# YonkaMayonkaZ/NCF

Measured on NVIDIA B200. Metric: NeuMF train samples/s, higher is better.
Workload: dtype f32

## Files before the change

ncf_b200/csrc/tile_umma.cu:

```cuda
#include <algorithm>
#include <cstdlib>

#include "common.cuh"
#include "tile_params.cuh"

namespace {

constexpr int kTile = 128;
constexpr uint32_t kHiMask = 0xffffe000u;
constexpr int kProducerWarps = 8;
constexpr int kLoaderWarp = 17;
constexpr int kGemmThreads = 576;
constexpr int kMaxStages = 4;

enum { EPI_RELU_STORE = 0, EPI_PREDICT = 1, EPI_PREDICT_TRAIN = 2, EPI_MASK_STORE = 3, EPI_SCATTER = 4 };

struct GemmArgs {
  int K;
  int N;
  int n_total;
  int passes;
  int layer;
  int gather;
  int stages;
  const float* a;
  const float* b_img;
  const float* bias;
  float* out;
  const float* mask_src;
};

struct WgradJob {
  int k, mb, nb, cta0, nctas;
  int S;
};
struct WgradArgs {
  int njobs, passes;
  WgradJob job[12];
};

__device__ __forceinline__ uint32_t smem_u32(const void* p) { return (uint32_t)__cvta_generic_to_shared(p); }

__device__ __forceinline__ void mbar_init(uint64_t* b, uint32_t count) {
  asm volatile("mbarrier.init.shared::cta.b64 [%0], %1;" ::"r"(smem_u32(b)), "r"(count));
}
__device__ __forceinline__ void mbar_arrive(uint64_t* b) {
  asm volatile("mbarrier.arrive.shared::cta.b64 _, [%0];" ::"r"(smem_u32(b)) : "memory");
}
__device__ __forceinline__ void mbar_expect_tx(uint64_t* b, uint32_t bytes) {
  asm volatile("mbarrier.arrive.expect_tx.shared::cta.b64 _, [%0], %1;" ::"r"(smem_u32(b)), "r"(bytes) : "memory");
}
__device__ __forceinline__ void mbar_wait(uint64_t* b, uint32_t parity) {
  const uint32_t addr = smem_u32(b);
  for (uint32_t spin = 0; spin < (1u << 26); ++spin) {
    uint32_t done;
#ifdef NCF_MBAR_POLL
    asm volatile(
        "{\n\t.reg .pred p;\n\tmbarrier.test_wait.parity.shared::cta.b64 p, [%1], %2;\n\tselp.u32 %0, 1, 0, p;\n\t}"
        : "=r"(done) : "r"(addr), "r"(parity) : "memory");
#else
    asm volatile(
        "{\n\t.reg .pred p;\n\tmbarrier.try_wait.parity.shared::cta.b64 p, [%1], %2;\n\tselp.u32 %0, 1, 0, p;\n\t}"
        : "=r"(done) : "r"(addr), "r"(parity) : "memory");
#endif
    if (done) return;
  }
  __trap();
}
__device__ __forceinline__ bool mbar_test_warp(uint64_t* b, uint32_t parity) {
  uint32_t done = 0;
  if ((threadIdx.x & 31) == 0)
    asm volatile(
        "{\n\t.reg .pred p;\n\tmbarrier.test_wait.parity.shared::cta.b64 p, [%1], %2;\n\tselp.u32 %0, 1, 0, p;\n\t}"
        : "=r"(done) : "r"(smem_u32(b)), "r"(parity) : "memory");
  return __shfl_sync(0xffffffffu, done, 0) != 0;
}
__device__ __forceinline__ void mbar_wait_warp(uint64_t* b, uint32_t parity) {
  if ((threadIdx.x & 31) == 0) mbar_wait(b, parity);
  __syncwarp();
}
__device__ __forceinline__ void mbar_arrive_warp(uint64_t* b) {
  __syncwarp();
  if ((threadIdx.x & 31) == 0) mbar_arrive(b);
}
__device__ __forceinline__ void bulk_g2s(void* dst, const void* src, uint32_t bytes, uint64_t* bar) {
  asm volatile("cp.async.bulk.shared::cluster.global.mbarrier::complete_tx::bytes [%0], [%1], %2, [%3];"
               ::"r"(smem_u32(dst)), "l"(src), "r"(bytes), "r"(smem_u32(bar)) : "memory");
}
__device__ __forceinline__ void cp_async16_zfill(void* dst, const void* src, bool valid) {
  asm volatile("cp.async.cg.shared.global [%0], [%1], 16, %2;" ::"r"(smem_u32(dst)), "l"(src), "r"(valid ? 16 : 0) : "memory");
}
__device__ __forceinline__ void fence_async_smem() { asm volatile("fence.proxy.async.shared::cta;" ::: "memory"); }
__device__ __forceinline__ void tc_fence_before() { asm volatile("tcgen05.fence::before_thread_sync;" ::: "memory"); }
__device__ __forceinline__ void tc_fence_after() { asm volatile("tcgen05.fence::after_thread_sync;" ::: "memory"); }
__device__ __forceinline__ void tc_commit(uint64_t* bar) {
  asm volatile("tcgen05.commit.cta_group::1.mbarrier::arrive::one.shared::cluster.b64 [%0];" ::"r"(smem_u32(bar)) : "memory");
}
__device__ __forceinline__ void tc_mma(uint32_t d_tmem, uint64_t da, uint64_t db, uint32_t idesc, uint32_t accumulate) {
  asm volatile(
      "{\n\t.reg .pred p;\n\tsetp.ne.b32 p, %4, 0;\n\t"
      "tcgen05.mma.cta_group::1.kind::tf32 [%0], %1, %2, %3, p;\n\t}"
      ::"r"(d_tmem), "l"(da), "l"(db), "r"(idesc), "r"(accumulate) : "memory");
}
__device__ __forceinline__ void tc_ld32(uint32_t taddr, float (&v)[32]) {
  uint32_t r[32];
  asm volatile(
      "tcgen05.ld.sync.aligned.32x32b.x32.b32 "
      "{%0,%1,%2,%3,%4,%5,%6,%7,%8,%9,%10,%11,%12,%13,%14,%15,"
      "%16,%17,%18,%19,%20,%21,%22,%23,%24,%25,%26,%27,%28,%29,%30,%31}, [%32];"
      : "=r"(r[0]), "=r"(r[1]), "=r"(r[2]), "=r"(r[3]), "=r"(r[4]), "=r"(r[5]), "=r"(r[6]), "=r"(r[7]),
        "=r"(r[8]), "=r"(r[9]), "=r"(r[10]), "=r"(r[11]), "=r"(r[12]), "=r"(r[13]), "=r"(r[14]), "=r"(r[15]),
        "=r"(r[16]), "=r"(r[17]), "=r"(r[18]), "=r"(r[19]), "=r"(r[20]), "=r"(r[21]), "=r"(r[22]), "=r"(r[23]),
        "=r"(r[24]), "=r"(r[25]), "=r"(r[26]), "=r"(r[27]), "=r"(r[28]), "=r"(r[29]), "=r"(r[30]), "=r"(r[31])
      : "r"(taddr));
  asm volatile("tcgen05.wait::ld.sync.aligned;" ::: "memory");
#pragma unroll
  for (int j = 0; j < 32; ++j) v[j] = __uint_as_float(r[j]);
}

__device__ __forceinline__ uint64_t make_desc(uint32_t addr, uint32_t lbo, uint32_t sbo, uint32_t layout) {
  uint64_t d = (uint64_t)(layout & 7) << 61;
  d |= (uint64_t)((addr >> 4) & 0x3fff);
  d |= (uint64_t)((lbo >> 4) & 0x3fff) << 16;
  d |= (uint64_t)((sbo >> 4) & 0x3fff) << 32;
  d |= (uint64_t)1 << 46;
  return d;
}
__device__ __forceinline__ uint32_t make_idesc(int m, int n, int a_mn, int b_mn) {
  uint32_t d = 0;
  d |= 1u << 4;
  d |= 2u << 7;
  d |= 2u << 10;
  d |= (uint32_t)a_mn << 15;
  d |= (uint32_t)b_mn << 16;
  d |= (uint32_t)(n >> 3) << 17;
  d |= (uint32_t)(m >> 4) << 24;
  return d;
}

__device__ __forceinline__ void split4(const float4 x, float4& hi, float4& lo) {
  hi.x = __uint_as_float(__float_as_uint(x.x) & kHiMask);
  hi.y = __uint_as_float(__float_as_uint(x.y) & kHiMask);
  hi.z = __uint_as_float(__float_as_uint(x.z) & kHiMask);
  hi.w = __uint_as_float(__float_as_uint(x.w) & kHiMask);
  lo = make_float4(x.x - hi.x, x.y - hi.y, x.z - hi.z, x.w - hi.w);
}

__device__ __forceinline__ float warp_colsum32(float (&v)[32], int lane) {
#pragma unroll
  for (int o = 16; o > 0; o >>= 1) {
    const bool upper = (lane & o) != 0;
#pragma unroll
    for (int i = 0; i < o; ++i) {
      const float send = upper ? v[i] : v[i + o];
      const float keep = upper ? v[i + o] : v[i];
      v[i] = keep + __shfl_xor_sync(0xffffffffu, send, o);
    }
  }
  return v[0];
}

__device__ __forceinline__ void named_bar(int id, int count) {
  asm volatile("bar.sync %0, %1;" ::"r"(id), "r"(count) : "memory");
}

__global__ void umma_weight_images_kernel(const TileParams p) {
  const int k = blockIdx.y >> 1, dir = blockIdx.y & 1;
  const int kin = p.W[k], nout = p.W[k + 1];
  const int rows = dir ? kin : nout, K = dir ? nout : kin;
  const int panels = (K + 31) / 32;
  const float* w = p.w[k];
  float* img = dir ? p.wsplit_b[k] : p.wsplit_f[k];
  const int64_t total = (int64_t)panels * rows * 32;
  for (int64_t idx = blockIdx.x * (int64_t)blockDim.x + threadIdx.x; idx < total;
       idx += (int64_t)gridDim.x * blockDim.x) {
    const int cc = (int)(idx & 31);
    const int r = (int)((idx >> 5) % rows);
    const int pi = (int)((idx >> 5) / rows);
    const int c = pi * 32 + cc;
    float x = 0.f;
    if (c < K) x = dir ? w[(int64_t)c * kin + r] : w[(int64_t)r * kin + c];
    const float hi = __uint_as_float(__float_as_uint(x) & kHiMask);
    const int64_t off = (int64_t)pi * 2 * rows * 32 + (int64_t)r * 32 + ((((cc >> 2) ^ (r & 7)) << 2) | (cc & 3));
    img[off] = hi;
    img[off + (int64_t)rows * 32] = x - hi;
  }
}
// ... 711 lines not shown
          } else if (TRAIN && ok && p.dlogit_in == nullptr) {
            pre_label = p.label[row];
            if (p.teacher != nullptr) pre_teacher = p.teacher[row];
          }
        }
        mbar_wait_warp(&bars.acc_ready[gi & 1], n_acc[gi & 1] & 1);
        ++n_acc[gi & 1];
        tc_fence_after();
        if (G.kind == 0 && G.k + 1 == L && hf == 1) bars.xch[q * 32 + lane] = gd;
        const bool zero_late = (gi + 1 == g.ng) && G.d_col == g.gemm[0].d_col;
        if (gi + 1 == g.ng) {
          if (!zero_late) {
            zero_cols(g.gemm[0].d_col, g.gemm[0].N);
            tc_wait_st();
          }
        } else if (g.gemm[gi + 1].new_operand) {
          for (int gj = gi + 1; gj < g.ng && (gj == gi + 1 || !g.gemm[gj].new_operand); ++gj)
            zero_cols(g.gemm[gj].d_col, g.gemm[gj].N);
          tc_wait_st();
          tc_fence_before();
          mbar_arrive_warp(&bars.opnd_ready);
        }
        const int N = G.N, k = G.k;
        const int nchunk = N >> 5;
        const int c_begin = (nchunk >= 2) ? hf * (nchunk / 2) * 32 : 0;
        const int c_end = (nchunk >= 2) ? (hf + 1) * (nchunk / 2) * 32 : (hf == 0 ? N : 0);
        if (G.kind == 0 && k + 1 == L) {
          const int trow = q * 32 + lane;
          if (hf == 0) {
            const float* bias = p.b[k];
            float acc = 0.f;
            for (int c0 = 0; c0 < N; c0 += 32) {
              tc_ld32(lane_addr + g.hcol[L] + c0, v);
#pragma unroll
              for (int j = 0; j < 32; ++j)
                acc = fmaf(__ldg(&p.pw[mlp_off + c0 + j]), fmaxf(v[j] + __ldg(&bias[c0 + j]), 0.f), acc);
            }
            named_bar(1 + q, 64);
            float x = acc + bars.xch[trow] + __ldg(p.pb);
            if (bad) x = __int_as_float(0x7fc00000);
            if (valid && p.logits != nullptr) p.logits[row] = x;
            if (TRAIN) {
              float ls = 0.f;
              if (ok && p.dlogit_in != nullptr) {
                dl = p.dlogit_in[row];
              } else if (ok) {
                const SampleLoss r = sample_loss(x, pre_label, p.teacher != nullptr, pre_teacher, p.alpha, p.invB);
                ls = r.loss;
                dl = r.dlogit;
              }
              bars.xch[trow] = dl;
              mbar_arrive_warp(&bars.dl_ready);
              const float ls_w = warp_sum(ls), dl_w = warp_sum(dl);
              if (lane == 0) {
                if (p.loss_accum != nullptr) atomicAdd(p.loss_accum, (double)ls_w * (double)p.invB);
                atomicAdd(&bars.pg[p.predict_size], dl_w);
              }
              for (int c0 = 0; c0 < N; c0 += 32) {
                tc_ld32(lane_addr + g.hcol[L] + c0, v);
                float z[32];
#pragma unroll
                for (int j = 0; j < 32; ++j) {
                  const float h = fmaxf(v[j] + __ldg(&bias[c0 + j]), 0.f);
                  z[j] = (h > 0.f) ? dl * __ldg(&p.pw[mlp_off + c0 + j]) : 0.f;
                  v[j] = dl * h;
                }
                tc_st32(lane_addr + g.hcol[L] + c0, z);
                const float s = warp_colsum32(v, lane);
                atomicAdd(&bars.pg[mlp_off + c0 + lane], s);
                if (g.passes == 3) {
#pragma unroll
                  for (int j = 0; j < 32; ++j) v[j] = lo_of(z[j]);
                  tc_st32(lane_addr + g.lcol[L] + c0, v);
                }
                quad8_transpose(z, lane);
                tc_wait_st();
                tc_fence_before();
                mbar_arrive_warp(&bars.panel_ready[c0 >> 5]);
                store_rows_t(z, p.delta[L], N, row - lane, p.B, c0, lane);
              }
            }
          } else {
            named_bar(1 + q, 64);
          }
        } else if (G.kind == 0) {
          const int kk = k + 1;
          const float* bias = p.b[k];
          for (int c0 = c_begin; c0 < c_end; c0 += 32) {
            tc_ld32(lane_addr + g.hcol[kk] + c0, v);
#pragma unroll
            for (int j = 0; j < 32; ++j) v[j] = fmaxf(v[j] + __ldg(&bias[c0 + j]), 0.f);
            tc_st32(lane_addr + g.hcol[kk] + c0, v);
            if (g.passes == 3) {
              float lo[32];
#pragma unroll
              for (int j = 0; j < 32; ++j) lo[j] = lo_of(v[j]);
              tc_st32(lane_addr + g.lcol[kk] + c0, lo);
            }
            if (TRAIN) quad8_transpose(v, lane);
            tc_wait_st();
            tc_fence_before();
            mbar_arrive_warp(&bars.panel_ready[c0 >> 5]);
            if (TRAIN) store_rows_t(v, p.act[kk], N, row - lane, p.B, c0, lane);
          }

        } else if (TRAIN && k > 0) {
          for (int c0 = c_begin; c0 < c_end; c0 += 32) {
            float x[32];
            tc_ld32(lane_addr + g.lcol[k] + c0, v);
            tc_ld32(lane_addr + g.hcol[k] + c0, x);
#pragma unroll
            for (int j = 0; j < 32; ++j) v[j] = (x[j] > 0.f) ? v[j] : 0.f;
            tc_st32(lane_addr + g.lcol[k] + c0, v);
            if (g.passes == 3) {
#pragma unroll
              for (int j = 0; j < 32; ++j) x[j] = lo_of(v[j]);
              tc_st32(lane_addr + g.hcol[k] + c0, x);
            }
            quad8_transpose(v, lane);
            tc_wait_st();
            tc_fence_before();
            mbar_arrive_warp(&bars.panel_ready[c0 >> 5]);
            store_rows_t(v, p.delta[k], N, row - lane, p.B, c0, lane);
          }
        } else if (TRAIN) {
          for (int c0 = c_begin; c0 < c_end; c0 += 32) {
            tc_ld32(lane_addr + G.d_col + c0, v);
            quad8_transpose(v, lane);
            const int col = G.row0 + c0;
            const bool to_user = col < dmlp;
            const int64_t my_idx = ok ? (to_user ? u : it) : -1;
            float* tab = (to_user ? p.gum + col : p.gim + (col - dmlp)) + 4 * (lane & 7);
#pragma unroll
            for (int i = 0; i < 8; ++i) {
              const int64_t idx = __shfl_sync(0xffffffffu, my_idx, (lane & ~7) + i);
              if (idx >= 0) red_add4(tab + idx * dmlp, make_float4(v[4 * i], v[4 * i + 1], v[4 * i + 2], v[4 * i + 3]));
            }
          }
        }
        if (zero_late) zero_cols(g.gemm[0].d_col, g.gemm[0].N);
        tc_wait_st();
        tc_fence_before();
        if (gi + 1 == g.ng) mbar_arrive_warp(&bars.tile_done);
      }
    }
  }
  tc_fence_before();
  __syncthreads();
  if (TRAIN)
    for (int i = tid; i <= p.predict_size; i += kTowerThreads) atomicAdd(&p.gt[p.pw_off + i], bars.pg[i]);
  if (warp == 8) asm volatile("tcgen05.dealloc.cta_group::1.sync.aligned.b32 %0, 512;" ::"r"(tmem));
}

constexpr int kWgProducerWarps = 8;
constexpr int kWgProducers = kWgProducerWarps * 32;
constexpr int kWgradThreads = kWgProducers + 96;

constexpr int kWgStages = 2;
struct WgradBars {
  uint64_t full[kWgStages], empty[kWgStages], acc_full;
  uint32_t tmem_base;
  float db[128];
};

__device__ __forceinline__ uint32_t mn_offset(int s, int fo, int S) {
  const int panel = fo >> 5, cc = fo & 31;
  return (uint32_t)(panel * (S * 128) + s * 128 + (((cc >> 3) ^ (s & 3)) << 5) + ((cc & 7) << 2));
}

__global__ void __launch_bounds__(kWgradThreads, 1)
umma_wgrad_kernel(const __grid_constant__ TileParams p, const __grid_constant__ WgradArgs g) {
  extern __shared__ __align__(1024) uint8_t smem_raw[];
  __shared__ WgradBars bars;
  uint8_t* smem = reinterpret_cast<uint8_t*>((reinterpret_cast<uintptr_t>(smem_raw) + 1023) & ~(uintptr_t)1023);
  const int tid = threadIdx.x, warp = tid >> 5, lane = tid & 31;
  int ji = 0;
  while (ji + 1 < g.njobs && (int)blockIdx.x >= g.job[ji + 1].cta0) ++ji;
  const WgradJob job = g.job[ji];
  const int k = job.k, kin = p.W[k], nout = p.W[k + 1];
  const int MB = min(128, nout - job.mb * 128), NB = min(256, kin - job.nb * 256);
  const int local = (int)blockIdx.x - job.cta0;
  const int S = job.S;
  const int64_t nchunks = (p.B + S - 1) / S;
  const uint32_t a_img = (uint32_t)MB * S * 4, b_img = (uint32_t)NB * S * 4;
  const uint32_t stage_bytes = 2 * a_img + 2 * b_img;
  const int64_t my_chunks = (local < nchunks) ? (nchunks - local + job.nctas - 1) / job.nctas : 0;

  if (tid == 0) {
    const int nm = (g.passes == 3) ? 3 : 1;
    for (int s = 0; s < kWgStages; ++s) { mbar_init(&bars.full[s], kWgProducerWarps); mbar_init(&bars.empty[s], nm); }
    mbar_init(&bars.acc_full, nm);
    asm volatile("fence.mbarrier_init.release.cluster;" ::: "memory");
  }
  if (tid < 128) bars.db[tid] = 0.f;
  if (warp == kWgProducerWarps) {
    asm volatile("tcgen05.alloc.cta_group::1.sync.aligned.shared::cta.b32 [%0], 256;" ::"r"(smem_u32(&bars.tmem_base)));
    asm volatile("tcgen05.relinquish_alloc_permit.cta_group::1.sync.aligned;");
  }
  tc_fence_before();
  __syncthreads();
  tc_fence_after();
  const uint32_t tmem = bars.tmem_base;
  if (warp < kWgProducerWarps) {
    float z[32];
#pragma unroll
    for (int j = 0; j < 32; ++j) z[j] = 0.f;
    for (int c0 = (warp >> 2) * 128; c0 < (warp >> 2) * 128 + 128; c0 += 32)
      tc_st32(tmem + ((uint32_t)((warp & 3) * 32) << 16) + c0, z);
    tc_wait_st();
  }
  tc_fence_before();
  __syncthreads();
  tc_fence_after();

  if (warp < kWgProducerWarps) {
    const int t = tid, d = p.d;
    const float* delta = p.delta[k + 1];
    const float* actk = (k > 0) ? p.act[k] : nullptr;
    const int pa = MB >> 2, pb = NB >> 2;
    const int na = S * pa / kWgProducers, nbp = S * pb / kWgProducers;
    const int ca = t % pa, sa0 = t / pa, sas = kWgProducers / pa;
    const int cb = t % pb, sb0 = t / pb, sbs = kWgProducers / pb;
    float4 dbsum = make_float4(0.f, 0.f, 0.f, 0.f);
    const int fo = job.nb * 256 + cb * 4;
    const bool from_user = fo < d;
    const int64_t* idx_src = from_user ? p.user : p.item;
    const float* tab = from_user ? p.eum + fo : p.eim + (fo - d);
    const int64_t idx_lim = from_user ? p.U : p.I;
    int64_t idx_even[8], idx_odd[8];
    auto issue_idx = [&](int64_t ci, int64_t (&idxv)[8]) {
      const int64_t row0 = (local + ci * job.nctas) * S;
#pragma unroll
      for (int i = 0; i < 8; ++i) {
        const int64_t row = row0 + sb0 + i * sbs;
        idxv[i] = (i < nbp && ci < my_chunks && row < p.B) ? idx_src[row] : -1;
      }
    };
    auto issue = [&](int64_t ci, bool blocking) -> bool {
      const int s = (int)(ci % kWgStages);
      const uint32_t par = (uint32_t)((ci / kWgStages) & 1) ^ 1;
      if (blocking) mbar_wait_warp(&bars.empty[s], par);
      else if (!mbar_test_warp(&bars.empty[s], par)) return false;
      uint8_t* st = smem + (size_t)s * stage_bytes;
      const int64_t row0 = (local + ci * job.nctas) * S;
#pragma unroll
      for (int i = 0; i < 4; ++i) {
        if (i < na) {
          const int64_t row = row0 + sa0 + i * sas;
          const bool ok = row < p.B;
          cp_async16_zfill(st + mn_offset(sa0 + i * sas, ca * 4, S),
                           ok ? delta + row * nout + job.mb * 128 + ca * 4 : delta, ok);
        }
      }
#pragma unroll
      for (int i = 0; i < 8; ++i) {
        if (i < nbp) {
          const float* src;
          bool ok;
          if (k == 0) {
            const int64_t ix = (ci & 1) ? idx_odd[i] : idx_even[i];
            ok = ix >= 0 && ix < idx_lim;
            src = ok ? tab + ix * d : tab;
          } else {
            const int64_t row = row0 + sb0 + i * sbs;
            ok = row < p.B;
            src = ok ? actk + row * kin + fo : actk;
          }
          cp_async16_zfill(st + 2 * a_img + mn_offset(sb0 + i * sbs, cb * 4, S), src, ok);
        }
      }
      asm volatile("cp.async.commit_group;" ::: "memory");
      if (k == 0) {
        if (ci & 1) issue_idx(ci + 2, idx_odd);
        else issue_idx(ci + 2, idx_even);
      }
      return true;
    };
    auto consume = [&](int64_t ci, int newer) {
      const int s = (int)(ci % kWgStages);
      uint8_t* st = smem + (size_t)s * stage_bytes;
      if (newer >= 3) asm volatile("cp.async.wait_group 3;" ::: "memory");
      else if (newer == 2) asm volatile("cp.async.wait_group 2;" ::: "memory");
      else if (newer == 1) asm volatile("cp.async.wait_group 1;" ::: "memory");
      else asm volatile("cp.async.wait_group 0;" ::: "memory");
#pragma unroll
      for (int i = 0; i < 4; ++i) {
        if (i < na) {
          const uint32_t off = mn_offset(sa0 + i * sas, ca * 4, S);
          const float4 x = *reinterpret_cast<const float4*>(st + off);
          float4 hi, lo;
          split4(x, hi, lo);
          dbsum.x += x.x; dbsum.y += x.y; dbsum.z += x.z; dbsum.w += x.w;
          if (g.passes == 3) *reinterpret_cast<float4*>(st + a_img + off) = lo;
        }
      }
#pragma unroll
      for (int i = 0; i < 8; ++i) {
        if (i < nbp && g.passes == 3) {
          const uint32_t off = 2 * a_img + mn_offset(sb0 + i * sbs, cb * 4, S);
          const float4 x = *reinterpret_cast<const float4*>(st + off);
          float4 hi, lo;
          split4(x, hi, lo);
          *reinterpret_cast<float4*>(st + b_img + off) = lo;
        }
      }
      fence_async_smem();
      mbar_arrive_warp(&bars.full[s]);
    };
    if (k == 0) {
      issue_idx(0, idx_even);
      issue_idx(1, idx_odd);
    }
    int64_t issued = 0;
    for (int64_t ci = 0; ci < my_chunks; ++ci) {
      if (issued == ci) issue(issued++, true);
      while (issued < my_chunks && issued - ci < kWgStages && issue(issued, false)) ++issued;
      consume(ci, (int)(issued - ci - 1));
    }
    if (job.nb == 0) {
      atomicAdd(&bars.db[ca * 4 + 0], dbsum.x);
      atomicAdd(&bars.db[ca * 4 + 1], dbsum.y);
      atomicAdd(&bars.db[ca * 4 + 2], dbsum.z);
      atomicAdd(&bars.db[ca * 4 + 3], dbsum.w);
    }
    named_bar(1, kWgProducers);
    if (job.nb == 0 && t < MB && my_chunks > 0) atomicAdd(&p.gt[p.b_off[k] + job.mb * 128 + t], bars.db[t]);
    if (my_chunks > 0) {
      mbar_wait_warp(&bars.acc_full, 0);
      tc_fence_after();
      const int q = warp & 3, part = warp >> 2, parts = min(kWgProducerWarps / 4, NB / 32);
      const int m = q * 32 + lane;
      float* dst = p.gt + p.w_off[k] + (int64_t)(job.mb * 128 + m) * kin + job.nb * 256;
      float v[32];
      for (int c0 = part * (NB / parts); c0 < (part + 1) * (NB / parts) && part < parts; c0 += 32) {
        tc_ld32(tmem + ((uint32_t)(q * 32) << 16) + c0, v);
        if (m < MB) {
#pragma unroll
          for (int j = 0; j < 32; j += 4) red_add4(dst + c0 + j, make_float4(v[j], v[j + 1], v[j + 2], v[j + 3]));
        }
      }
    }
  } else if (lane == 0 && (warp == kWgProducerWarps || g.passes == 3)) {
    const int pass = warp - kWgProducerWarps;
    const uint32_t idesc = make_idesc(128, NB, 1, 1);
    for (int64_t ci = 0; ci < my_chunks; ++ci) {
      const int s = (int)(ci % kWgStages);
      mbar_wait(&bars.full[s], (uint32_t)(ci / kWgStages) & 1);
      tc_fence_after();
      const uint32_t base = smem_u32(smem + (size_t)s * stage_bytes);
      const uint32_t ahi = base, alo = base + a_img, bhi = base + 2 * a_img, blo = bhi + b_img;
      const uint64_t da0 = make_desc(pass == 1 ? alo : ahi, S * 128, 512, 1);
      const uint64_t db0 = make_desc(pass == 2 ? blo : bhi, S * 128, 512, 1);
      for (int ks = 0; ks < S / 8; ++ks) tc_mma(tmem, da0 + 64 * ks, db0 + 64 * ks, idesc, 1u);
      tc_commit(&bars.empty[s]);
    }
    if (my_chunks > 0) tc_commit(&bars.acc_full);
  }
  tc_fence_before();
  __syncthreads();
  if (warp == kWgProducerWarps) asm volatile("tcgen05.dealloc.cta_group::1.sync.aligned.b32 %0, 256;" ::"r"(tmem));
}

constexpr size_t kSmemBudget = 200 * 1024;

template <int EPI>
int launch_gemm(const TileParams& p, GemmArgs g, int nblocks, cudaStream_t st) {
  const size_t stage = 2 * (size_t)kTile * 128 + 2 * (size_t)g.N * 128;
  int stages = (int)(kSmemBudget / stage);
  if (stages > kMaxStages) stages = kMaxStages;
  if (stages < 2) {
    ncf::set_error("umma gemm: stage of %zu bytes does not fit twice", stage);
    return NCF_ERR_ARG;
  }
  g.stages = stages;
  const size_t smem = stages * stage + 1024;
  auto kern = umma_gemm_kernel<EPI>;
  NCF_CUDA(cudaFuncSetAttribute(kern, cudaFuncAttributeMaxDynamicSharedMemorySize, (int)smem));
  const int64_t ntiles = (p.B + kTile - 1) / kTile;
  int64_t grid = ncf::num_sms();
  if (grid > ntiles) grid = ntiles;
  kern<<<dim3((unsigned)grid, (unsigned)nblocks), kGemmThreads, smem, st>>>(p, g);
  NCF_LAUNCH_CHECK("umma_gemm_kernel");
  return NCF_OK;
}

int launch_wgrad(const TileParams& p, int passes, cudaStream_t st) {
  WgradArgs g{};
  g.passes = passes;
  double weight[12], total = 0;
  for (int k = 0; k < p.L; ++k) {
    const int mbs = (p.W[k + 1] + 127) / 128, nbs = (p.W[k] + 255) / 256;
    for (int mb = 0; mb < mbs; ++mb)
      for (int nb = 0; nb < nbs; ++nb) {
        if (g.njobs >= 12) {
          ncf::set_error("umma wgrad: too many weight blocks");
          return NCF_ERR_ARG;
        }
        const int MB = std::min(128, p.W[k + 1] - mb * 128), NB = std::min(256, p.W[k] - nb * 256);
        int S = std::min(4096 / MB, 8192 / NB) / 8 * 8;
        S = std::max(8, std::min(S, 256));
        g.job[g.njobs] = WgradJob{k, mb, nb, 0, 0, S};
        weight[g.njobs] = 1.0 / S;
        total += weight[g.njobs];
        ++g.njobs;
      }
  }
  const int sms = ncf::num_sms();
  int cta = 0;
  size_t smem = 0;
  for (int j = 0; j < g.njobs; ++j) {
    const int64_t nchunks = (p.B + g.job[j].S - 1) / g.job[j].S;
    int n = (int)(weight[j] / total * sms);
    if (n < 1) n = 1;
    if (n > nchunks) n = (int)nchunks;
    g.job[j].cta0 = cta;
    g.job[j].nctas = n;
    cta += n;
    const int k = g.job[j].k;
    const int MB = std::min(128, p.W[k + 1] - g.job[j].mb * 128), NB = std::min(256, p.W[k] - g.job[j].nb * 256);
    smem = std::max(smem, (size_t)kWgStages * 2 * (MB + NB) * g.job[j].S * 4);
  }
  smem += 1024;
  NCF_CUDA(cudaFuncSetAttribute(umma_wgrad_kernel, cudaFuncAttributeMaxDynamicSharedMemorySize, (int)smem));
  umma_wgrad_kernel<<<cta, kWgradThreads, smem, st>>>(p, g);
  NCF_LAUNCH_CHECK("umma_wgrad_kernel");
  return NCF_OK;
}

struct StepProfile {
  int enabled = 0, n = 0;
  float ms[16];
  const char* name[16];
};
thread_local StepProfile g_profile;

struct StepTimer {
  bool on;
  cudaStream_t st;
  cudaEvent_t ev[32];
  const char* name[32];
  int n = 0;
  static thread_local StepTimer* g_timer;
  StepTimer(cudaStream_t s) : on(g_profile.enabled), st(s) {
    g_timer = this;
    mark("start");
  }
  void mark(const char* what) {
    if (!on || n >= 32) return;
    cudaEventCreate(&ev[n]);
    cudaEventRecord(ev[n], st);
    name[n++] = what;
  }
  ~StepTimer() {
    g_timer = nullptr;
    if (!on) return;
    cudaStreamSynchronize(st);
    g_profile.n = 0;
    for (int i = 1; i < n; ++i) {
      float ms = 0;
      cudaEventElapsedTime(&ms, ev[i - 1], ev[i]);
      if (g_profile.n < 16) {
        g_profile.ms[g_profile.n] = ms;
        g_profile.name[g_profile.n++] = name[i];
      }
    }
    for (int i = 0; i < n; ++i) cudaEventDestroy(ev[i]);
  }
};

thread_local StepTimer* StepTimer::g_timer = nullptr;

GemmArgs forward_args(const TileParams& p, int k, int passes) {
  GemmArgs g{};
  g.K = p.W[k];
  g.n_total = p.W[k + 1];
  g.N = std::min(256, g.n_total);
  g.passes = passes;
  g.layer = k;
  g.gather = (k == 0);
  g.a = (k == 0) ? nullptr : p.act[k];
  g.b_img = p.wsplit_f[k];
  g.bias = p.b[k];
  return g;
}

int tower_forward(TileParams& p, int passes, bool train, cudaStream_t st) {
  for (int k = 0; k < p.L; ++k) {
    GemmArgs g = forward_args(p, k, passes);
    int rc;
    if (k + 1 < p.L) {
      g.out = p.act[k + 1];
      rc = launch_gemm<EPI_RELU_STORE>(p, g, g.n_total / g.N, st);
    } else if (train) {
      g.out = p.delta[p.L];
      rc = launch_gemm<EPI_PREDICT_TRAIN>(p, g, 1, st);
    } else {
      rc = launch_gemm<EPI_PREDICT>(p, g, 1, st);
    }
    if (rc != NCF_OK) return rc;
    if (StepTimer::g_timer) StepTimer::g_timer->mark(k == 0 ? "fwd0" : k == 1 ? "fwd1" : "fwd2+");
  }
  return NCF_OK;
}

bool tower_fused_ok(const TileParams& p) {
  const char* off = getenv("NCF_UMMA_FUSED");
  if (off != nullptr && off[0] == '0') return false;
  if (p.W[0] > 256 || p.W[p.L] < 32 || p.f > 64) return false;
  int cols = 0;
  for (int k = 1; k <= p.L; ++k) cols += 2 * p.W[k];
  return cols <= 512 && 2 * p.W[1] + p.W[0] <= 512;
}

template <bool TRAIN>
int launch_tower(const TileParams& p, int passes, cudaStream_t st) {
  TowerArgs g{};
  g.passes = passes;
  int col = 0;
  for (int k = 1; k <= p.L; ++k) {
    g.hcol[k] = col;
    col += p.W[k];
    g.lcol[k] = col;
    col += p.W[k];
  }
  g.ring_col = p.W[1];
  g.ring_stages = std::min(kRingMax, (512 - p.W[1]) / 64);
  for (int k = 0; k < p.L; ++k)
    g.gemm[g.ng++] = TowerGemm{0, k, p.W[k + 1], p.W[k], k == 0 ? -1 : g.hcol[k], k == 0 ? -1 : g.lcol[k],
                               g.hcol[k + 1], p.W[k + 1], 0, k > 0, p.wsplit_f[k]};
  if (TRAIN)
    for (int k = p.L - 1; k >= 0; --k) {
      const bool top = (k + 1 == p.L);
      const int a_hi = top ? g.hcol[p.L] : g.lcol[k + 1], a_lo = top ? g.lcol[p.L] : g.hcol[k + 1];
      for (int n0 = 0; n0 < p.W[k]; n0 += 128) {
        const int N = std::min(128, p.W[k] - n0);
        g.gemm[g.ng++] = TowerGemm{1, k, N, p.W[k + 1], a_hi, a_lo, (k >= 1 ? g.lcol[k] : 2 * p.W[1]) + n0,
                                   p.W[k], n0, n0 == 0, p.wsplit_b[k]};
      }
    }
  const size_t smem = (size_t)kBStages * 128 * 256 + (size_t)(p.W[0] / 32) * kTile * 128 + 1024;
  auto kern = umma_tower_kernel<TRAIN>;
  NCF_CUDA(cudaFuncSetAttribute(kern, cudaFuncAttributeMaxDynamicSharedMemorySize, (int)smem));
  const int64_t ntiles = (p.B + kTile - 1) / kTile;
  int64_t grid = ncf::num_sms();
  if (grid > ntiles) grid = ntiles;
  kern<<<(unsigned)grid, kTowerThreads, smem, st>>>(p, g);
  NCF_LAUNCH_CHECK("umma_tower_kernel");
  return NCF_OK;
}

}

namespace ncf {

bool umma_eligible(const TileParams& p) {
  const char* off = getenv("NCF_UMMA_DISABLE");
  if (off != nullptr && off[0] == '1') return false;
  const char* mb = getenv("NCF_UMMA_MIN_B");
  const int64_t min_b = mb ? atoll(mb) : 8192;
  if (p.B < min_b) return false;
  if (p.type == NCF_GMF) return false;
  if (p.f < 32 || p.f > 128 || (p.f & (p.f - 1)) != 0) return false;
  int blocks = 0;
  for (int k = 0; k < p.L; ++k) blocks += ((p.W[k + 1] + 127) / 128) * ((p.W[k] + 255) / 256);
  return blocks <= 12;
}

int64_t umma_image_floats(const TileParams& p) {
  int64_t n = 0;
  for (int k = 0; k < p.L; ++k) n += 2 * 2 * (int64_t)p.W[k] * p.W[k + 1];
  return n;
}

// ... 121 lines not shown
```

Baseline: 166.5 million.

## Stage wgrad delta operand in tensor memory and decouple A/B pipelines

The weight-gradient kernel now has dedicated delta warps that read delta columns per lane and store them, with their hi/lo split, straight into tensor memory. The MMA then uses the TMEM-A form (tc_mma_ts), and A and B get separate multi-stage mbarrier pipelines. Bias-gradient reduction moves into those warps. This drops the shared-memory round trip and the in-smem split for the delta operand and frees smem for deeper activation staging. The costs are a 512-column TMEM allocation, a smaller fixed chunk S, new fit constraints that reject some shapes, and strided per-lane global loads of delta.

Result: slower. 122.5 million (median of 6 runs) (-26.4%).

```diff
diff --git a/ncf_b200/csrc/tile_umma.cu b/ncf_b200/csrc/tile_umma.cu
--- a/ncf_b200/csrc/tile_umma.cu
+++ b/ncf_b200/csrc/tile_umma.cu
@@ -33,6 +33,7 @@
 struct WgradJob {
   int k, mb, nb, cta0, nctas;
   int S;
+  int stages_a, stages_b;
 };
 struct WgradArgs {
   int njobs, passes;
@@ -1050,15 +1051,17 @@
   if (warp == 8) asm volatile("tcgen05.dealloc.cta_group::1.sync.aligned.b32 %0, 512;" ::"r"(tmem));
 }
 
-constexpr int kWgProducerWarps = 8;
-constexpr int kWgProducers = kWgProducerWarps * 32;
-constexpr int kWgradThreads = kWgProducers + 96;
-
-constexpr int kWgStages = 2;
+constexpr int kWgDeltaWarps = 4;
+constexpr int kWgActWarp0 = kWgDeltaWarps;
+constexpr int kWgActThreads = 8 * 32;
+constexpr int kWgMmaWarp = kWgActWarp0 + kWgActThreads / 32;
+constexpr int kWgradThreads = (kWgMmaWarp + 3) * 32;
+constexpr int kWgTmemCols = 512;
+constexpr int kWgMaxStagesA = 4, kWgMaxStagesB = 4;
+
 struct WgradBars {
-  uint64_t full[kWgStages], empty[kWgStages], acc_full;
+  uint64_t a_full[kWgMaxStagesA], a_empty[kWgMaxStagesA], b_full[kWgMaxStagesB], b_empty[kWgMaxStagesB], acc_full;
   uint32_t tmem_base;
-  float db[128];
 };
 
 __device__ __forceinline__ uint32_t mn_offset(int s, int fo, int S) {
@@ -1078,48 +1081,95 @@
   const int k = job.k, kin = p.W[k], nout = p.W[k + 1];
   const int MB = min(128, nout - job.mb * 128), NB = min(256, kin - job.nb * 256);
   const int local = (int)blockIdx.x - job.cta0;
-  const int S = job.S;
+  const int S = job.S, SA = job.stages_a, SB = job.stages_b;
+  const int nq = MB >> 5;
   const int64_t nchunks = (p.B + S - 1) / S;
-  const uint32_t a_img = (uint32_t)MB * S * 4, b_img = (uint32_t)NB * S * 4;
-  const uint32_t stage_bytes = 2 * a_img + 2 * b_img;
+  const uint32_t b_img = (uint32_t)NB * S * 4, b_stage = 2 * b_img;
+  const uint32_t a_cols = (g.passes == 3) ? 2 * S : S;
   const int64_t my_chunks = (local < nchunks) ? (nchunks - local + job.nctas - 1) / job.nctas : 0;
 
   if (tid == 0) {
     const int nm = (g.passes == 3) ? 3 : 1;
-    for (int s = 0; s < kWgStages; ++s) { mbar_init(&bars.full[s], kWgProducerWarps); mbar_init(&bars.empty[s], nm); }
+    for (int s = 0; s < SA; ++s) { mbar_init(&bars.a_full[s], nq); mbar_init(&bars.a_empty[s], nm); }
+    for (int s = 0; s < SB; ++s) { mbar_init(&bars.b_full[s], kWgActThreads / 32); mbar_init(&bars.b_empty[s], nm); }
     mbar_init(&bars.acc_full, nm);
     asm volatile("fence.mbarrier_init.release.cluster;" ::: "memory");
   }
-  if (tid < 128) bars.db[tid] = 0.f;
-  if (warp == kWgProducerWarps) {
-    asm volatile("tcgen05.alloc.cta_group::1.sync.aligned.shared::cta.b32 [%0], 256;" ::"r"(smem_u32(&bars.tmem_base)));
+  if (warp == kWgMmaWarp) {
+    asm volatile("tcgen05.alloc.cta_group::1.sync.aligned.shared::cta.b32 [%0], 512;" ::"r"(smem_u32(&bars.tmem_base)));
     asm volatile("tcgen05.relinquish_alloc_permit.cta_group::1.sync.aligned;");
   }
   tc_fence_before();
   __syncthreads();
   tc_fence_after();
   const uint32_t tmem = bars.tmem_base;
-  if (warp < kWgProducerWarps) {
+  {
     float z[32];
 #pragma unroll
     for (int j = 0; j < 32; ++j) z[j] = 0.f;
-    for (int c0 = (warp >> 2) * 128; c0 < (warp >> 2) * 128 + 128; c0 += 32)
-      tc_st32(tmem + ((uint32_t)((warp & 3) * 32) << 16) + c0, z);
+    const uint32_t lane_addr = tmem + ((uint32_t)((warp & 3) * 32) << 16);
+    if (warp >= kWgActWarp0 && warp < kWgMmaWarp) {
+      const int c_begin = ((warp - kWgActWarp0) >> 2) * 128;
+      for (int c0 = c_begin; c0 < min(NB, c_begin + 128); c0 += 32) tc_st32(lane_addr + c0, z);
+    } else if (warp < kWgDeltaWarps && warp >= nq) {
+      for (int c0 = NB; c0 < NB + SA * (int)a_cols; c0 += 32) tc_st32(lane_addr + c0, z);
+    }
     tc_wait_st();
   }
   tc_fence_before();
   __syncthreads();
   tc_fence_after();
 
-  if (warp < kWgProducerWarps) {
-    const int t = tid, d = p.d;
-    const float* delta = p.delta[k + 1];
+  if (warp < kWgDeltaWarps) {
+    if (warp < nq && my_chunks > 0) {
+      const int m = warp * 32 + lane;
+      const float* col = p.delta[k + 1] + job.mb * 128 + m;
+      const uint32_t lane_addr = tmem + ((uint32_t)(warp * 32) << 16) + NB;
+      const int groups = S >> 5;
+      float nxt[32], dsum = 0.f;
+      auto load = [&](int64_t ci, int h) {
+        const int64_t row0 = (local + ci * job.nctas) * S + h * 32;
+#pragma unroll
+        for (int j = 0; j < 32; ++j) {
+          const int64_t row = row0 + j;
+          nxt[j] = (ci < my_chunks && row < p.B) ? __ldg(col + row * nout) : 0.f;
+        }
+      };
+      load(0, 0);
+      for (int64_t ci = 0; ci < my_chunks; ++ci) {
+        const int s = (int)(ci % SA);
+        for (int h = 0; h < groups; ++h) {
+          float v[32];
+#pragma unroll
+          for (int j = 0; j < 32; ++j) v[j] = nxt[j];
+          if (h + 1 < groups) load(ci, h + 1);
+          else load(ci + 1, 0);
+          if (h == 0) {
+            mbar_wait_warp(&bars.a_empty[s], (uint32_t)((ci / SA) & 1) ^ 1);
+            tc_fence_after();
+          }
+          const uint32_t a = lane_addr + s * a_cols + h * 32;
+          tc_st32(a, v);
+#pragma unroll
+          for (int j = 0; j < 32; ++j) dsum += v[j];
+          if (g.passes == 3) {
+#pragma unroll
+            for (int j = 0; j < 32; ++j) v[j] = lo_of(v[j]);
+            tc_st32(a + S, v);
+          }
+        }
+        tc_wait_st();
+        tc_fence_before();
+        mbar_arrive_warp(&bars.a_full[s]);
+      }
+      if (job.nb == 0) atomicAdd(&p.gt[p.b_off[k] + job.mb * 128 + m], dsum);
+    }
+  } else if (warp < kWgMmaWarp) {
+    const int t = tid - kWgActWarp0 * 32, d = p.d;
     const float* actk = (k > 0) ? p.act[k] : nullptr;
-    const int pa = MB >> 2, pb = NB >> 2;
-    const int na = S * pa / kWgProducers, nbp = S * pb / kWgProducers;
-    const int ca = t % pa, sa0 = t / pa, sas = kWgProducers / pa;
-    const int cb = t % pb, sb0 = t / pb, sbs = kWgProducers / pb;
-    float4 dbsum = make_float4(0.f, 0.f, 0.f, 0.f);
+    const int pb = NB >> 2;
+    const int nbp = S * pb / kWgActThreads;
+    const int cb = t % pb, sb0 = t / pb, sbs = kWgActThreads / pb;
     const int fo = job.nb * 256 + cb * 4;
     const bool from_user = fo < d;
     const int64_t* idx_src = from_user ? p.user : p.item;
@@ -1135,21 +1185,12 @@
       }
     };
     auto issue = [&](int64_t ci, bool blocking) -> bool {
-      const int s = (int)(ci % kWgStages);
-      const uint32_t par = (uint32_t)((ci / kWgStages) & 1) ^ 1;
-      if (blocking) mbar_wait_warp(&bars.empty[s], par);
-      else if (!mbar_test_warp(&bars.empty[s], par)) return false;
-      uint8_t* st = smem + (size_t)s * stage_bytes;
+      const int s = (int)(ci % SB);
+      const uint32_t par = (uint32_t)((ci / SB) & 1) ^ 1;
+      if (blocking) mbar_wait_warp(&bars.b_empty[s], par);
+      else if (!mbar_test_warp(&bars.b_empty[s], par)) return false;
+      uint8_t* st = smem + (size_t)s * b_stage;
       const int64_t row0 = (local + ci * job.nctas) * S;
-#pragma unroll
-      for (int i = 0; i < 4; ++i) {
-        if (i < na) {
-          const int64_t row = row0 + sa0 + i * sas;
-          const bool ok = row < p.B;
-          cp_async16_zfill(st + mn_offset(sa0 + i * sas, ca * 4, S),
-                           ok ? delta + row * nout + job.mb * 128 + ca * 4 : delta, ok);
-        }
-      }
 #pragma unroll
       for (int i = 0; i < 8; ++i) {
         if (i < nbp) {
@@ -1164,7 +1205,7 @@
             ok = row < p.B;
             src = ok ? actk + row * kin + fo : actk;
           }
-          cp_async16_zfill(st + 2 * a_img + mn_offset(sb0 + i * sbs, cb * 4, S), src, ok);
+          cp_async16_zfill(st + mn_offset(sb0 + i * sbs, cb * 4, S), src, ok);
         }
       }
       asm volatile("cp.async.commit_group;" ::: "memory");
@@ -1175,35 +1216,25 @@
       return true;
     };
     auto consume = [&](int64_t ci, int newer) {
-      const int s = (int)(ci % kWgStages);
-      uint8_t* st = smem + (size_t)s * stage_bytes;
+      uint8_t* st = smem + (size_t)(ci % SB) * b_stage;
       if (newer >= 3) asm volatile("cp.async.wait_group 3;" ::: "memory");
       else if (newer == 2) asm volatile("cp.async.wait_group 2;" ::: "memory");
       else if (newer == 1) asm volatile("cp.async.wait_group 1;" ::: "memory");
       else asm volatile("cp.async.wait_group 0;" ::: "memory");
-#pragma unroll
-      for (int i = 0; i < 4; ++i) {
-        if (i < na) {
-          const uint32_t off = mn_offset(sa0 + i * sas, ca * 4, S);
-          const float4 x = *reinterpret_cast<const float4*>(st + off);
-          float4 hi, lo;
-          split4(x, hi, lo);
-          dbsum.x += x.x; dbsum.y += x.y; dbsum.z += x.z; dbsum.w += x.w;
-          if (g.passes == 3) *reinterpret_cast<float4*>(st + a_img + off) = lo;
-        }
-      }
-#pragma unroll
-      for (int i = 0; i < 8; ++i) {
-        if (i < nbp && g.passes == 3) {
-          const uint32_t off = 2 * a_img + mn_offset(sb0 + i * sbs, cb * 4, S);
-          const float4 x = *reinterpret_cast<const float4*>(st + off);
-          float4 hi, lo;
-          split4(x, hi, lo);
-          *reinterpret_cast<float4*>(st + b_img + off) = lo;
+      if (g.passes == 3) {
+#pragma unroll
+        for (int i = 0; i < 8; ++i) {
+          if (i < nbp) {
+            const uint32_t off = mn_offset(sb0 + i * sbs, cb * 4, S);
+            const float4 x = *reinterpret_cast<const float4*>(st + off);
+            float4 hi, lo;
+            split4(x, hi, lo);
+            *reinterpret_cast<float4*>(st + b_img + off) = lo;
+          }
         }
       }
       fence_async_smem();
-      mbar_arrive_warp(&bars.full[s]);
+      mbar_arrive_warp(&bars.b_full[ci % SB]);
     };
     if (k == 0) {
       issue_idx(0, idx_even);
@@ -1212,21 +1243,13 @@
     int64_t issued = 0;
     for (int64_t ci = 0; ci < my_chunks; ++ci) {
       if (issued == ci) issue(issued++, true);
-      while (issued < my_chunks && issued - ci < kWgStages && issue(issued, false)) ++issued;
+      while (issued < my_chunks && issued - ci < SB && issue(issued, false)) ++issued;
       consume(ci, (int)(issued - ci - 1));
     }
-    if (job.nb == 0) {
-      atomicAdd(&bars.db[ca * 4 + 0], dbsum.x);
-      atomicAdd(&bars.db[ca * 4 + 1], dbsum.y);
-      atomicAdd(&bars.db[ca * 4 + 2], dbsum.z);
-      atomicAdd(&bars.db[ca * 4 + 3], dbsum.w);
-    }
-    named_bar(1, kWgProducers);
-    if (job.nb == 0 && t < MB && my_chunks > 0) atomicAdd(&p.gt[p.b_off[k] + job.mb * 128 + t], bars.db[t]);
     if (my_chunks > 0) {
       mbar_wait_warp(&bars.acc_full, 0);
       tc_fence_after();
-      const int q = warp & 3, part = warp >> 2, parts = min(kWgProducerWarps / 4, NB / 32);
+      const int q = warp & 3, part = (warp - kWgActWarp0) >> 2, parts = min(2, NB / 32);
       const int m = q * 32 + lane;
       float* dst = p.gt + p.w_off[k] + (int64_t)(job.mb * 128 + m) * kin + job.nb * 256;
       float v[32];
@@ -1238,25 +1261,26 @@
         }
       }
     }
-  } else if (lane == 0 && (warp == kWgProducerWarps || g.passes == 3)) {
-    const int pass = warp - kWgProducerWarps;
-    const uint32_t idesc = make_idesc(128, NB, 1, 1);
+  } else if (lane == 0 && (warp == kWgMmaWarp || g.passes == 3)) {
+    const int pass = warp - kWgMmaWarp;
+    const uint32_t idesc = make_idesc(128, NB, 0, 1);
     for (int64_t ci = 0; ci < my_chunks; ++ci) {
-      const int s = (int)(ci % kWgStages);
-      mbar_wait(&bars.full[s], (uint32_t)(ci / kWgStages) & 1);
+      const int sa = (int)(ci % SA), sb = (int)(ci % SB);
+      mbar_wait(&bars.a_full[sa], (uint32_t)(ci / SA) & 1);
+      mbar_wait(&bars.b_full[sb], (uint32_t)(ci / SB) & 1);
       tc_fence_after();
-      const uint32_t base = smem_u32(smem + (size_t)s * stage_bytes);
-      const uint32_t ahi = base, alo = base + a_img, bhi = base + 2 * a_img, blo = bhi + b_img;
-      const uint64_t da0 = make_desc(pass == 1 ? alo : ahi, S * 128, 512, 1);
-      const uint64_t db0 = make_desc(pass == 2 ? blo : bhi, S * 128, 512, 1);
-      for (int ks = 0; ks < S / 8; ++ks) tc_mma(tmem, da0 + 64 * ks, db0 + 64 * ks, idesc, 1u);
-      tc_commit(&bars.empty[s]);
+      const uint32_t a = tmem + NB + sa * a_cols + (pass == 1 ? S : 0);
+      const uint32_t bhi = smem_u32(smem + (size_t)sb * b_stage);
+      const uint64_t db0 = make_desc(pass == 2 ? bhi + b_img : bhi, S * 128, 512, 1);
+      for (int ks = 0; ks < S / 8; ++ks) tc_mma_ts(tmem, a + 8 * ks, db0 + 64 * ks, idesc, 1u);
+      tc_commit(&bars.a_empty[sa]);
+      tc_commit(&bars.b_empty[sb]);
     }
     if (my_chunks > 0) tc_commit(&bars.acc_full);
   }
   tc_fence_before();
   __syncthreads();
-  if (warp == kWgProducerWarps) asm volatile("tcgen05.dealloc.cta_group::1.sync.aligned.b32 %0, 256;" ::"r"(tmem));
+  if (warp == kWgMmaWarp) asm volatile("tcgen05.dealloc.cta_group::1.sync.aligned.b32 %0, 512;" ::"r"(tmem));
 }
 
 constexpr size_t kSmemBudget = 200 * 1024;
@@ -1285,7 +1309,9 @@
 int launch_wgrad(const TileParams& p, int passes, cudaStream_t st) {
   WgradArgs g{};
   g.passes = passes;
+  constexpr size_t kStageBudget = 225 * 1024;
   double weight[12], total = 0;
+  size_t smem = 0;
   for (int k = 0; k < p.L; ++k) {
     const int mbs = (p.W[k + 1] + 127) / 128, nbs = (p.W[k] + 255) / 256;
     for (int mb = 0; mb < mbs; ++mb)
@@ -1295,17 +1321,24 @@
           return NCF_ERR_ARG;
         }
         const int MB = std::min(128, p.W[k + 1] - mb * 128), NB = std::min(256, p.W[k] - nb * 256);
-        int S = std::min(4096 / MB, 8192 / NB) / 8 * 8;
-        S = std::max(8, std::min(S, 256));
-        g.job[g.njobs] = WgradJob{k, mb, nb, 0, 0, S};
-        weight[g.njobs] = 1.0 / S;
+        const int S = std::min(64, 8192 / std::max(NB, 1));
+        const int a_cols = (passes == 3 ? 2 : 1) * S;
+        const size_t b_stage = 2 * (size_t)NB * S * 4;
+        const int sa = std::min(kWgMaxStagesA, (kWgTmemCols - NB) / a_cols);
+        const int sb = (int)std::min<size_t>(kWgMaxStagesB, kStageBudget / b_stage);
+        if (MB % 32 != 0 || NB % 32 != 0 || S % 32 != 0 || sa < 2 || sb < 2) {
+          ncf::set_error("umma wgrad: block %d x %d of layer %d does not fit (S %d, stages %d / %d)", MB, NB, k, S, sa, sb);
+          return NCF_ERR_ARG;
+        }
+        g.job[g.njobs] = WgradJob{k, mb, nb, 0, 0, S, sa, sb};
+        smem = std::max(smem, sb * b_stage);
+        weight[g.njobs] = MB + NB;
         total += weight[g.njobs];
         ++g.njobs;
       }
   }
   const int sms = ncf::num_sms();
   int cta = 0;
-  size_t smem = 0;
   for (int j = 0; j < g.njobs; ++j) {
     const int64_t nchunks = (p.B + g.job[j].S - 1) / g.job[j].S;
     int n = (int)(weight[j] / total * sms);
@@ -1314,9 +1347,6 @@
     g.job[j].cta0 = cta;
     g.job[j].nctas = n;
     cta += n;
-    const int k = g.job[j].k;
-    const int MB = std::min(128, p.W[k + 1] - g.job[j].mb * 128), NB = std::min(256, p.W[k] - g.job[j].nb * 256);
-    smem = std::max(smem, (size_t)kWgStages * 2 * (MB + NB) * g.job[j].S * 4);
   }
   smem += 1024;
   NCF_CUDA(cudaFuncSetAttribute(umma_wgrad_kernel, cudaFuncAttributeMaxDynamicSharedMemorySize, (int)smem));
```
